# mvenouziou/Boosted_DETR

Measured on AMD Instinct MI355X. Metric: images/sec training step (fwd+matcher+loss+bwd), 640x640 N=100, higher is better.
Workload: dtype f32 (conv/GEMM products as 3 split-f16 [fwd] / split-bf16 [grad] MFMA products, f32 accumulate)

## Files before the change

### boosted_detr_amd/_lib.py

```python
from __future__ import annotations

import ctypes as C
import os
from pathlib import Path

_LIB_PATH = Path(os.environ.get("BDETR_LIB") or Path(__file__).resolve().parent / "csrc" / "libbdetr.so")
_lib = None

c_f32p = C.c_void_p
c_i32p = C.c_void_p
c_i64p = C.c_void_p
c_stream = C.c_void_p


class ConvDesc(C.Structure):
    _fields_ = [(n, C.c_int) for n in ("N", "H", "W", "C", "K", "R", "S", "stride", "pad", "OH", "OW")]


class GemmDesc(C.Structure):
    _fields_ = [
        ("I", C.c_int), ("J", C.c_int), ("R", C.c_int), ("nb0", C.c_int), ("nb1", C.c_int),
        ("a", C.c_void_p), ("lda", C.c_int64), ("sa0", C.c_int64), ("sa1", C.c_int64), ("a_rcontig", C.c_int),
        ("b", C.c_void_p), ("ldb", C.c_int64), ("sb0", C.c_int64), ("sb1", C.c_int64), ("b_rcontig", C.c_int),
        ("c", C.c_void_p), ("ldc", C.c_int64), ("sc0", C.c_int64), ("sc1", C.c_int64),
# ... 12 lines not shown
                ("y2", C.c_void_p), ("mean2", C.c_void_p), ("rstd2", C.c_void_p), ("part_gx2", C.c_void_p)]


class RowchainFwdDesc(C.Structure):
    _fields_ = ([("M", C.c_int64), ("nstages", C.c_int), ("eps", C.c_float), ("rate", C.c_float), ("ctx", C.c_void_p), ("resid", C.c_void_p),
                 ("w", C.c_void_p * 3), ("bias", C.c_void_p * 3)]
                + [(n, C.c_void_p) for n in ("g1", "b1", "g2", "b2", "pre1", "x1", "mean1", "rstd1", "h", "pre2", "x2", "mean2", "rstd2")]
                + [("seed1", C.c_uint64), ("seed2", C.c_uint64), ("seed_base", C.c_void_p)])


class RowchainBwdDesc(C.Structure):
    _fields_ = ([("M", C.c_int64), ("nstages", C.c_int), ("rate", C.c_float)]
                + [(n, C.c_void_p) for n in ("dout", "pre2", "mean2", "rstd2", "g2", "h", "pre1", "mean1", "rstd1", "g1")]
                + [("wt", C.c_void_p * 3)]
                + [(n, C.c_void_p) for n in ("G2", "G1", "G0", "dresid", "dctx", "partials")]
                + [("seed1", C.c_uint64), ("seed2", C.c_uint64), ("seed_base", C.c_void_p)])


class LossDesc(C.Structure):
    _fields_ = [("B", C.c_int), ("M", C.c_int), ("N", C.c_int), ("C", C.c_int), ("A", C.c_int),
                ("category_weight", C.c_float), ("attribute_weight", C.c_float),
                ("box_weight", C.c_float), ("exist_weight", C.c_float)]


P = C.c_void_p
I = C.c_int
L = C.c_int64
F = C.c_float
U64 = C.c_uint64

SIGNATURES = {
    "bdetr_abi_version": (I, []),
    "bdetr_last_error": (C.c_char_p, []),
    "bdetr_device_cus": (I, []),
    "bdetr_low_priority_stream_create": (I, [P]),
    "bdetr_side_stream_candidates": (I, [P, I, I, I, P, P, P]),
    "bdetr_stream_destroy": (I, [P]),
    "bdetr_stream_priority_range": (I, [P, P]),
    "bdetr_set_gemm_precision": (I, [I]),
    "bdetr_get_gemm_precision": (I, []),
    "bdetr_prof_enable": (I, [I]),
    "bdetr_prof_read": (I, [P, P, P]),
    "bdetr_prof_read_arith": (I, [I, P, P, P]),
    "bdetr_prof_dump": (I, [C.c_char_p]),
    "bdetr_image_prep": (I, [P, I, I, I, P, I, I, P]),
    "bdetr_tokens_prepare": (I, [P, P, L, I, I, I, P, P, P]),
    "bdetr_augment_ws_floats": (I, [I]),
    "bdetr_augment": (I, [P, P, P, P, I, I, I, P, P]),
    "bdetr_jpeg_quality_ws_bytes": (C.c_int64, [I, I, I]),
    "bdetr_jpeg_quality": (I, [P, P, P, I, I, I, P, P]),
    "bdetr_augment_jpeg": (I, [P, P, P, P, P, I, I, I, P, P, P]),
    "bdetr_conv2d_fwd": (I, [P, P, P, P, C.POINTER(ConvDesc), I, P, P, P]),
    "bdetr_conv2d_fwd_stat_chunks": (I, [C.POINTER(ConvDesc)]),
    "bdetr_conv2d_bwd_data": (I, [P, P, P, C.POINTER(ConvDesc), I, P]),
    "bdetr_conv2d_bwd_weight": (I, [P, P, P, C.POINTER(ConvDesc), I, P]),
    "bdetr_conv2d_bwd_weight_splitk": (I, [C.POINTER(ConvDesc)]),
    "bdetr_bn_apply_p16": (I, [P, P, P, P, P, P, I, C.POINTER(BnAffine), I, P, P, P, P, P, L, I, P]),
    "bdetr_bn_bwd_p16": (I, [P, P, I, P, P, P, P, P, I, I, P, P, P, P, P, P, P, P, I, L, I, P]),
    "bdetr_bn_bwd_p16_even_pixels": (I, [P, P, I, P, P, P, P, P, I, I, P, P, P, P, P, P, I, I, I, I, I, P]),
    "bdetr_p16_supported": (I, [C.POINTER(ConvDesc)]),
    "bdetr_p16_pack": (I, [P, L, P, P, P, P]),
    "bdetr_p16_unpack": (I, [P, I, L, P, P]),
    "bdetr_p16_pack_conv_weights": (I, [P, I, I, I, I, P, P, P, P]),
    "bdetr_p16_pack_conv_weights_multi": (I, [P, I, P, P]),
    "bdetr_p16_conv2d_fwd_stat_chunks": (I, [C.POINTER(ConvDesc)]),
    "bdetr_p16_conv2d_fwd": (I, [P, P, P, P, C.POINTER(ConvDesc), I, P, P, P]),
    "bdetr_p16_conv2d_bwd_data": (I, [P, P, P, C.POINTER(ConvDesc), I, P]),
    "bdetr_p16_conv2d_bwd_data_stat_chunks": (I, [C.POINTER(ConvDesc)]),
    "bdetr_p16_conv2d_bwd_data_masked_accum": (I, [P, P, P, P, C.POINTER(ConvDesc), C.POINTER(BnBwdFuse), P]),
    "bdetr_p16_conv2d_bwd_data_masked_accum_compact": (I, [P, P, P, P, P, C.POINTER(ConvDesc), C.POINTER(BnBwdFuse), P]),
    "bdetr_relu_mask_apply": (I, [P, P, C.c_int64, P]),
    "bdetr_p16_conv2d_bwd_data_bnstats": (I, [P, P, P, C.POINTER(ConvDesc), C.POINTER(BnBwdFuse), P]),
    "bdetr_p16_conv2d_bwd_weight_splitk": (I, [C.POINTER(ConvDesc)]),
    "bdetr_p16_conv2d_bwd_weight": (I, [P, P, P, C.POINTER(ConvDesc), I, P]),
    "bdetr_p16_conv2d_bwd_weight_xf16": (I, [P, P, P, C.POINTER(ConvDesc), I, P]),
    "bdetr_gemm": (I, [C.POINTER(GemmDesc), P]),
    "bdetr_gemm_ws": (I, [C.POINTER(GemmDesc), P, L, P]),
    "bdetr_splitk_workspace_elems": (L, [L, L, I]),
    "bdetr_conv2d_bwd_weight_ws": (I, [P, P, P, C.POINTER(ConvDesc), I, P, L, P]),
    "bdetr_p16_conv2d_bwd_weight_ws": (I, [P, I, P, P, C.POINTER(ConvDesc), I, P, L, P]),
    "bdetr_gemm_grouped": (I, [C.POINTER(GemmDesc), I, P]),
    "bdetr_colsum_chunks": (I, [L]),
    "bdetr_colsum": (I, [P, L, I, P, P, P]),
    "bdetr_colsum_accumulate": (I, [P, L, I, P, P]),
    "bdetr_colsum_accumulate_group": (I, [P, P, I, P, I, P]),
    "bdetr_colstats": (I, [P, L, I, P, P, P]),
    "bdetr_bn_stats": (I, [P, L, I, P, P, I, F, F, I, P, P, P, P, P, P, P]),
    "bdetr_flag_nonfinite": (I, [P, L, P, P]),
    "bdetr_flag_snapshot": (I, [P, P, P, I, P]),
    "bdetr_debug_checksum": (I, [P, L, P, P, P, I, U64, P]),
    "bdetr_graph_node_census": (I, [P, P, I]),
    "bdetr_bn_stats_fold_rows": (I, []),
    "bdetr_bn_stats_frozen": (I, [P, P, I, F, P, P, P]),
    "bdetr_bn_apply": (I, [P, P, P, P, P, P, I, P, L, I, P]),
    "bdetr_bn_bwd_chunks": (I, [L]),
    "bdetr_bn_bwd": (I, [P, P, P, P, P, P, P, I, I, P, P, P, P, P, L, I, P]),
    "bdetr_bn_rows_stats": (I, [P, I, L, I, F, P, P, P, P, P]),
    "bdetr_bn_rows_apply": (I, [P, P, P, P, P, P, I, L, I, I, P, F, P, P, P, P]),
    "bdetr_bn_rows_bwd": (I, [P, P, P, P, P, I, I, P, P, P, P, I, L, I, P]),
    "bdetr_maxpool3x3s2_fwd": (I, [P, P, I, I, I, I, I, I, P]),
    "bdetr_maxpool3x3s2_bwd": (I, [P, P, P, P, I, I, I, I, I, I, P]),
    "bdetr_stem_pool_bwd_chunks": (I, [L]),
    "bdetr_stem_pool_fwd": (I, [P, P, P, P, P, I, I, I, I, P, P, P, P, P]),
    "bdetr_stem_pool_bwd": (I, [P, P, P, P, P, P, P, I, I, I, I, P, I, P, P, P, P]),
    "bdetr_p16_s2d_pack_bf16": (I, [P, I, I, I, P, P]),
    "bdetr_p16_stem_bwd_weight": (I, [P, P, P, I, I, I, I, P]),
# ... 101 lines not shown
```

### boosted_detr_amd/csrc/igemm.hip

```cpp
#include "gemm_common.h"
#include <stdlib.h>
#include <string.h>
#include <type_traits>
#include <utility>
#include <vector>

using namespace bdgemm;

namespace {

constexpr int BK = 32;
constexpr int RPAD = 4;
constexpr int NTHREADS = 256;

constexpr int SLD = 36;
constexpr int SLD3 = 52;
constexpr float LO_SCALE = 2048.f;
typedef __bf16 bf16x2 __attribute__((ext_vector_type(2)));
typedef __bf16 bf16x8 __attribute__((ext_vector_type(8)));
typedef _Float16 f16x2 __attribute__((ext_vector_type(2)));
typedef _Float16 f16x8 __attribute__((ext_vector_type(8)));
typedef float f32x2 __attribute__((ext_vector_type(2)));

template <int ARITH>
__device__ __forceinline__ void split2(float x0, float x1, unsigned& hi, unsigned& lo) {
    f32x2 v; v[0] = x0; v[1] = x1;
    if (ARITH == AR_BF16X3) {
        hi = __builtin_bit_cast(unsigned, __builtin_convertvector(v, bf16x2));
        f32x2 r;
        r[0] = x0 - __builtin_bit_cast(float, hi << 16);
        r[1] = x1 - __builtin_bit_cast(float, hi & 0xFFFF0000u);
        lo = __builtin_bit_cast(unsigned, __builtin_convertvector(r, bf16x2));
    } else {
        const f16x2 h = __builtin_convertvector(v, f16x2);
        hi = __builtin_bit_cast(unsigned, h);
        const f32x2 r = (v - __builtin_convertvector(h, f32x2)) * LO_SCALE;
        lo = __builtin_bit_cast(unsigned, __builtin_convertvector(r, f16x2));
    }
}

__device__ __forceinline__ void split3(float x0, float x1, unsigned& hi, unsigned& mid, unsigned& lo) {
    f32x2 v; v[0] = x0; v[1] = x1;
    hi = __builtin_bit_cast(unsigned, __builtin_convertvector(v, bf16x2));
    f32x2 r;
    r[0] = x0 - __builtin_bit_cast(float, hi << 16);
    r[1] = x1 - __builtin_bit_cast(float, hi & 0xFFFF0000u);
    mid = __builtin_bit_cast(unsigned, __builtin_convertvector(r, bf16x2));
    r[0] -= __builtin_bit_cast(float, mid << 16);
    r[1] -= __builtin_bit_cast(float, mid & 0xFFFF0000u);
    lo = __builtin_bit_cast(unsigned, __builtin_convertvector(r, bf16x2));
}

struct DenseOp { const float* p; int64_t ld, s0, s1; int rows, cols; };
// ... 358 lines not shown
#pragma unroll
            for (int e = 0; e < 4; ++e)
#pragma unroll
                for (int a = 0; a < TM; ++a)
#pragma unroll
                    for (int b = 0; b < TN; ++b)
                        acc[a][b] = __builtin_amdgcn_mfma_f32_32x32x2f32(fa[a][e], fb[b][e], acc[a][b], 0, 0, 0);
        }
    };

    const int nk = (r_end - r_begin + BK - 1) / BK;
    constexpr bool PF1 = SPLIT && BM * BN >= 128 * 128;
    if constexpr (PF1) {
        if (nk > 0) { load_stage(r_begin, stA0, stB0); write_stage(0, stA0, stB0); }
        __syncthreads();
        for (int kt = 0; kt < nk; ++kt) {
            if (kt + 1 < nk) load_stage(r_begin + (kt + 1) * BK, stA0, stB0);
            compute(kt & 1);
            if (kt + 1 < nk) write_stage((kt + 1) & 1, stA0, stB0);
            __syncthreads();
        }
    } else {
    if (nk > 0) {
        load_stage(r_begin, stA0, stB0);
        if (nk > 1) load_stage(r_begin + BK, stA1, stB1);
        write_stage(0, stA0, stB0);
    }
    __syncthreads();

    for (int kt = 0; kt < nk; kt += 2) {
        if (kt + 2 < nk) load_stage(r_begin + (kt + 2) * BK, stA0, stB0);
        compute(0);
        if (kt + 1 < nk) write_stage(1, stA1, stB1);
        __syncthreads();
        if (kt + 1 >= nk) break;
        if (kt + 3 < nk) load_stage(r_begin + (kt + 3) * BK, stA1, stB1);
        compute(1);
        if (kt + 2 < nk) write_stage(0, stA0, stB0);
        __syncthreads();
    }
    }

    if constexpr (ARITH == AR_FP16X3) {
#pragma unroll
        for (int a = 0; a < TM; ++a)
#pragma unroll
            for (int b = 0; b < TN; ++b)
#pragma unroll
                for (int e = 0; e < 16; ++e) acc[a][b][e] += acc2[a][b][e] * (1.f / LO_SCALE);
    }
    gemm_epilogue<BM, BN, WM, WN, NTHREADS, 2 * STAGE_FLOATS>(acc, g, lds, tile_i, i0, j0, g.c + (int64_t)(sk_ ? zz_ : b0) * g.sc0 + (int64_t)b1 * g.sc1);
}

struct TileChoice { int bm, bn; };

}

namespace bdgemm {
int g_num_cus = 0;
int num_cus() {
    if (g_num_cus == 0) {
        int dev = 0; hipDeviceProp_t p;
        if (hipGetDevice(&dev) == hipSuccess && hipGetDeviceProperties(&p, dev) == hipSuccess) g_num_cus = p.multiProcessorCount;
        if (g_num_cus <= 0) g_num_cus = 256;
    }
    return g_num_cus;
}
}

namespace {

}
namespace bdgemm {
thread_local int g_gemm_mode = -1;
int gemm_mode() {
    if (g_gemm_mode < 0) {
        const char* e = getenv("BDETR_GEMM_PRECISION");
        g_gemm_mode = !e ? BDETR_GEMM_MIXED : (!strcmp(e, "fp32") || !strcmp(e, "f32")) ? BDETR_GEMM_FP32
                    : !strcmp(e, "bf16x3") ? BDETR_GEMM_BF16X3 : !strcmp(e, "split") ? BDETR_GEMM_SPLIT : !strcmp(e, "bf16x6") ? BDETR_GEMM_BF16X6 : BDETR_GEMM_MIXED;
    }
    return g_gemm_mode;
}
}
namespace {
int use_split(bool grad) {
    switch (gemm_mode()) {
        case BDETR_GEMM_FP32:   return AR_FP32;
        case BDETR_GEMM_BF16X3: return AR_BF16X3;
        case BDETR_GEMM_SPLIT:  return grad ? AR_BF16X3 : AR_FP16X3;
        case BDETR_GEMM_BF16X6: return AR_BF16X6;
        default:                return grad ? AR_BF16X3 : AR_FP32;
    }
}

TileChoice choose_tile(int I, int J, int zdim, bool both_rc, bool split, bool patch = false) {
    static int forced_bm = -1, forced_bn = -1;
    if (forced_bm < 0) {
        forced_bm = forced_bn = 0;
        if (const char* e = getenv("BDETR_TILE")) sscanf(e, "%dx%d", &forced_bm, &forced_bn);
    }
    if (forced_bm > 0) {
        if (J <= 32) return {128, 32};
        return {forced_bm, forced_bn};
    }
    auto tiles = [&](int bm, int bn) { return cdiv64(I, bm) * cdiv64(J, bn) * zdim; };
    if (J <= 32) return {128, 32};
// ... 261 lines not shown
            if (arc && brc)   return launch_any<DenseLoader<4>, true, DenseLoader<4>, true>(a, b, g, zdim, st, sp);
            if (arc && !brc)  return launch_any<DenseLoader<4>, true, DenseLoader<4>, false>(a, b, g, zdim, st, sp);
            if (!arc && !brc) return launch_any<DenseLoader<4>, false, DenseLoader<4>, false>(a, b, g, zdim, st, sp);
            return launch_any<DenseLoader<4>, false, DenseLoader<4>, true>(a, b, g, zdim, st, sp, true);
        }
        if (arc && brc)   return launch_any<DenseLoader<1>, true, DenseLoader<1>, true>(a, b, g, zdim, st, AR_FP32, true);
        if (arc && !brc)  return launch_any<DenseLoader<1>, true, DenseLoader<1>, false>(a, b, g, zdim, st, AR_FP32, true);
        if (!arc && !brc) return launch_any<DenseLoader<1>, false, DenseLoader<1>, false>(a, b, g, zdim, st, AR_FP32, true);
        return launch_any<DenseLoader<1>, false, DenseLoader<1>, true>(a, b, g, zdim, st, AR_FP32, true);
    };
    if (ws != nullptr && splitk > 1) return with_splitk_slabs(g, zdim, ws, ws_elems, st, "bdetr_gemm_ws", launch);
    return launch();
}

static int check_conv(const bdetr_conv_desc* d, const char* who) {
    BDETR_CHECK_ARG(d != nullptr, "%s: null desc", who);
    BDETR_CHECK_ARG(d->N > 0 && d->H > 0 && d->W > 0 && d->C > 0 && d->K > 0 && d->R > 0 && d->S > 0 && d->stride > 0 && d->pad >= 0,
                    "%s: bad conv geometry", who);
    BDETR_CHECK_ARG(d->C % 4 == 0, "%s: input channels must be a multiple of 4 (got %d)", who, d->C);
    BDETR_CHECK_ARG(d->OH == (d->H + 2 * d->pad - d->R) / d->stride + 1 && d->OW == (d->W + 2 * d->pad - d->S) / d->stride + 1,
                    "%s: OH/OW inconsistent with geometry", who);
    BDETR_CHECK_ARG((int64_t)d->N * d->OH * d->OW < (1LL << 31) && (int64_t)d->R * d->S * d->C < (1LL << 31), "%s: problem too large", who);
    BDETR_CHECK_ARG(span_ok((int64_t)d->N * d->H * d->W * d->C) && span_ok((int64_t)d->N * d->OH * d->OW * d->K) && span_ok((int64_t)d->K * d->R * d->S * d->C),
                    "%s: a tensor spans 4 GB or more (the loaders use 32-bit buffer offsets); use a smaller per-GPU batch", who);
    return 0;
}

extern "C" int bdetr_conv2d_fwd_stat_chunks(const bdetr_conv_desc* d) {
    if (check_conv(d, "bdetr_conv2d_fwd_stat_chunks")) return -1;
    return stat_chunks(d->N * d->OH * d->OW, d->K);
}

extern "C" int bdetr_conv2d_fwd(const float* x, const float* w, const float* bias, float* y,
                                const bdetr_conv_desc* d, int act, float* stat_sum, float* stat_sq, void* stream) {
    if (int e = check_conv(d, "bdetr_conv2d_fwd")) return e;
    BDETR_CHECK_ARG(x && w && y, "bdetr_conv2d_fwd: null pointer");
    BDETR_CHECK_ARG(aligned16(x) && aligned16(w), "bdetr_conv2d_fwd: x and w must be 16-byte aligned");
    BDETR_CHECK_ARG((stat_sum == nullptr) == (stat_sq == nullptr), "bdetr_conv2d_fwd: stat_sum/stat_sq must both be set or both null");
    const int M = d->N * d->OH * d->OW, Kd = d->R * d->S * d->C;
    GemmParams g; init_params(g);
    g.I = M; g.J = d->K; g.R = Kd;
    g.c = y; g.ldc = d->K; g.bias = bias; g.act = act;
    g.stat_sum = stat_sum; g.stat_sq = stat_sq;
    DenseOp wop{w, Kd, 0, 0, d->K, Kd};
    hipStream_t st = (hipStream_t)stream;
    if (d->R == 1 && d->S == 1 && d->stride == 1 && d->pad == 0) {
        DenseOp xop{x, d->C, 0, 0, M, d->C};
        return launch_any<DenseLoader<4>, true, DenseLoader<4>, true>(xop, wop, g, 1, st, use_split(false));
    }
    PatchOp xop{x, d->N, d->H, d->W, d->C, d->OH, d->OW, d->R, d->S, d->stride, d->pad, M, Kd};
    return launch_any<PatchLoader, true, DenseLoader<4>, true>(xop, wop, g, 1, st, use_split(false));
}

extern "C" int bdetr_conv2d_bwd_data(const float* dy, const float* w, float* dx,
                                     const bdetr_conv_desc* d, int accumulate, void* stream) {
    if (int e = check_conv(d, "bdetr_conv2d_bwd_data")) return e;
    BDETR_CHECK_ARG(dy && w && dx, "bdetr_conv2d_bwd_data: null pointer");
    BDETR_CHECK_ARG(d->K % 4 == 0, "bdetr_conv2d_bwd_data: output channels must be a multiple of 4");
    hipStream_t st = (hipStream_t)stream;
    const int M = d->N * d->OH * d->OW;
    GemmParams g; init_params(g);
    g.c = dx; g.ldc = d->C; g.mode = accumulate ? ST_ACCUM : ST_STORE;
    if (d->R == 1 && d->S == 1 && d->pad == 0) {
        g.I = M; g.J = d->C; g.R = d->K;
        if (d->stride > 1) {
            if (!accumulate) {
                if (int e = bdetr_zero_bytes(dx, sizeof(float) * (size_t)d->N * d->H * d->W * d->C, st)) return e;
            }
            g.rowmap = 1; g.rm_OW = d->OW; g.rm_OHOW = d->OH * d->OW; g.rm_H = d->H; g.rm_W = d->W; g.rm_stride = d->stride;
        }
        DenseOp a{dy, d->K, 0, 0, M, d->K};
        DenseOp b{w, d->C, 0, 0, d->K, d->C};
        return launch_any<DenseLoader<4>, true, DenseLoader<4>, false>(a, b, g, 1, st, use_split(true));
    }
    if (d->stride > 1 && d->pad == 0 && d->R <= d->stride && d->S <= d->stride) {
        if (!accumulate) {
            if (int e = bdetr_zero_bytes(dx, sizeof(float) * (size_t)d->N * d->H * d->W * d->C, st)) return e;
        }
        g.I = M; g.J = d->C; g.R = d->K;
        g.rowmap = 1; g.rm_OW = d->OW; g.rm_OHOW = d->OH * d->OW; g.rm_H = d->H; g.rm_W = d->W; g.rm_stride = d->stride;
        DenseOp a{dy, d->K, 0, 0, M, d->K};
        for (int r = 0; r < d->R; ++r)
            for (int s = 0; s < d->S; ++s) {
                g.rm_off = r * d->W + s;
                DenseOp b{w + (int64_t)(r * d->S + s) * d->C, (int64_t)d->R * d->S * d->C, 0, 0, d->K, d->C};
                if (int e = launch_any<DenseLoader<4>, true, DenseLoader<4>, false>(a, b, g, 1, st, use_split(true))) return e;
            }
        return 0;
    }
    BDETR_CHECK_ARG(d->stride == 1, "bdetr_conv2d_bwd_data: stride>1 only for 1x1 convs or taps that do not overlap (R, S <= stride, pad 0)");
    const int Mx = d->N * d->H * d->W;
    g.I = Mx; g.J = d->C; g.R = d->R * d->S * d->K;
    PatchOp a{dy, d->N, d->OH, d->OW, d->K, d->H, d->W, d->R, d->S, 1, d->R - 1 - d->pad, Mx, d->R * d->S * d->K};
    BDETR_CHECK_ARG(d->R == d->S, "bdetr_conv2d_bwd_data: square kernels only");
    WFlipOp b{w, d->K, d->C, d->R, d->S, d->R * d->S * d->K, d->C};
    return launch_any<PatchLoader, true, WFlipLoader, false>(a, b, g, 1, st, use_split(true));
}

extern "C" int bdetr_conv2d_bwd_weight_splitk(const bdetr_conv_desc* d) {
    if (check_conv(d, "bdetr_conv2d_bwd_weight_splitk")) return -1;
    const int M = d->N * d->OH * d->OW, Kd = d->R * d->S * d->C;
    TileChoice t = choose_tile(d->K, Kd, 2, false, use_split(true) != AR_FP32, !(d->R == 1 && d->S == 1 && d->stride == 1 && d->pad == 0));
    int64_t tiles = cdiv64(d->K, t.bm) * cdiv64(Kd, t.bn);
    int64_t want = 3LL * num_cus();
    const bool few_tiles = tiles <= 8 && M >= (1 << 20);
    if (few_tiles) want = 16LL * num_cus();
// ... 43 lines not shown
```

### boosted_detr_amd/kernels.py

```python
from __future__ import annotations

import ctypes as C
from dataclasses import dataclass
from typing import Optional, Tuple

import numpy as np
import torch

from . import _lib
from ._lib import BnAffine, BnBwdFuse, ConvDesc, GemmDesc, LossDesc, RowchainBwdDesc, RowchainFwdDesc, check

ACT_NONE, ACT_RELU, ACT_TANH = 0, 1, 2


_LAUNCH_STREAM = [None]


def set_launch_stream(handle: Optional[int]) -> Optional[int]:
    prev = _LAUNCH_STREAM[0]
    _LAUNCH_STREAM[0] = handle
    return prev


GEMM_FP32, GEMM_BF16X3, GEMM_MIXED, GEMM_SPLIT, GEMM_BF16X6 = 0, 1, 2, 3, 4
# ... 124 lines not shown
    _chk(image)
    _chk(quality, dtype=torch.int32)
    B, H, W, c = image.shape
    assert c == 3 and quality.numel() == B
    L = _lib.lib()
    out = torch.empty_like(image)
    jws = torch.empty(int(L.bdetr_jpeg_quality_ws_bytes(B, H, W)), dtype=torch.uint8, device=image.device)
    check(L.bdetr_jpeg_quality(_p(image), _p(out), _p(quality), B, H, W, _p(jws), _stream()), "jpeg_quality")
    return out


@dataclass(frozen=True)
class ConvGeom:
    N: int
    H: int
    W: int
    C: int
    K: int
    R: int
    S: int
    stride: int
    pad: int

    @property
    def OH(self) -> int:
        return (self.H + 2 * self.pad - self.R) // self.stride + 1

    @property
    def OW(self) -> int:
        return (self.W + 2 * self.pad - self.S) // self.stride + 1

    @property
    def M(self) -> int:
        return self.N * self.OH * self.OW

    def desc(self) -> ConvDesc:
        return ConvDesc(self.N, self.H, self.W, self.C, self.K, self.R, self.S, self.stride, self.pad, self.OH, self.OW)


def conv2d_fwd(x, w, bias, g: ConvGeom, act: int = ACT_NONE, want_stats: bool = False):
    _chk(x, w, bias)
    L = _lib.lib()
    d = g.desc()
    y = empty(g.N, g.OH, g.OW, g.K, like=x)
    psum = psq = None
    nparts = 0
    if want_stats:
        nparts = L.bdetr_conv2d_fwd_stat_chunks(C.byref(d))
        if nparts <= 0:
            check(-1, "conv2d_fwd_stat_chunks")
        psum = empty(nparts, g.K, like=x)
        psq = empty(nparts, g.K, like=x)
    check(L.bdetr_conv2d_fwd(_p(x), _p(w), _p(bias), _p(y), C.byref(d), act, _p(psum), _p(psq), _stream()), "conv2d_fwd")
    return y, (psum, psq, nparts)


def conv2d_bwd_data(dy, w, g: ConvGeom, dx: Optional[torch.Tensor] = None, accumulate: bool = False):
    _chk(dy, w, dx)
    d = g.desc()
    if dx is None:
        assert not accumulate
        dx = empty(g.N, g.H, g.W, g.C, like=dy)
    check(_lib.lib().bdetr_conv2d_bwd_data(_p(dy), _p(w), _p(dx), C.byref(d), int(accumulate), _stream()), "conv2d_bwd_data")
    return dx


def conv2d_bwd_weight(x, dy, g: ConvGeom, dw: Optional[torch.Tensor] = None, prezeroed: bool = False):
    _chk(x, dy, dw)
    L = _lib.lib()
    d = g.desc()
    if dw is None:
        dw = empty(g.K, g.R, g.S, g.C, like=x)
        prezeroed = False
    sk = L.bdetr_conv2d_bwd_weight_splitk(C.byref(d))
    if sk > 1 and not prezeroed:
        check(L.bdetr_zero(_p(dw), dw.numel(), _stream()), "zero")
    ws, n = _splitk_ws(g.K, g.R * g.S * g.C, sk, x)
    check(L.bdetr_conv2d_bwd_weight_ws(_p(x), _p(dy), _p(dw), C.byref(d), sk, _p(ws), n, _stream()), "conv2d_bwd_weight")
    return dw


_OVERFLOW = [None]


def overflow_flag() -> torch.Tensor:
    if _OVERFLOW[0] is None:
        _OVERFLOW[0] = torch.zeros(1, dtype=torch.int32, device="cuda")
    return _OVERFLOW[0]


_GUARD_ACTIVE = [True]


def set_guard_active(on: bool) -> None:
    _GUARD_ACTIVE[0] = bool(on)


def flag_nonfinite(x: torch.Tensor) -> None:
    _chk(x)
    check(_lib.lib().bdetr_flag_nonfinite(_p(x), x.numel(), _p(overflow_flag()), _stream()), "flag_nonfinite")


def flag_snapshot(ordinal: torch.Tensor, host_ring: torch.Tensor) -> None:
    assert host_ring.dtype == torch.int32 and host_ring.numel() >= 2 and host_ring.is_pinned()
    assert ordinal.dtype == torch.int32 and ordinal.is_cuda
    check(_lib.lib().bdetr_flag_snapshot(_p(overflow_flag()), _p(ordinal), host_ring.data_ptr(), host_ring.numel() - 1, _stream()), "flag_snapshot")
# ... 1229 lines not shown
```

### boosted_detr_amd/ops.py

```python
from __future__ import annotations

import math
import os
import weakref
from typing import Optional

import numpy as np
import torch

from . import kernels as K
from . import _lib
from .engine import WEIGHTS_VERSION, Variable, capture, current_tape, dense_contribution, info, materialise, own, side_task, tag

_dropout_site = [0]
_dropout_seed_dev = [None]


def dropout_seed_tensor() -> torch.Tensor:
    if _dropout_seed_dev[0] is None:
        _dropout_seed_dev[0] = torch.full((1,), 0x5EED, dtype=torch.int64, device="cuda")
    return _dropout_seed_dev[0]


def set_dropout_seed(seed: int, write: bool = True) -> None:
# ... 433 lines not shown
    def backward(g_out):
        dx, _ = _bn_backward(_2d(g_out.contiguous()), None, x2d, mean, rstd, bn, False, not training, False)
        return (own(dx.view(x.shape)),)

    _rec([out], [x], backward)
    return out


def batchnorm_rows(x: torch.Tensor, bn: BNState, training: bool, groups: int) -> torch.Tensor:
    x2d = _2d(x)
    g, b = bn.gamma.value, bn.beta.value
    if training:
        mean, rstd, var = K.bn_rows_stats(x2d, groups, bn.eps)
        out2d = K.bn_rows_apply(x2d, groups, mean, rstd, g, b, var, bn.momentum, bn.moving_mean.value, bn.moving_var.value)
    else:
        K.demote_split_forward()
        mean, rstd = K.bn_stats_frozen(bn.moving_mean.value, bn.moving_var.value, bn.eps)
        out2d = K.bn_rows_apply(x2d, groups, mean, rstd, g, b)
    out = out2d.view(x.shape)

    def backward(g_out):
        sg, sb = GradSink(bn.gamma), GradSink(bn.beta)
        dx, _, _ = K.bn_rows_bwd(_2d(g_out.contiguous()), x2d, groups, mean, rstd, bn.gamma.value, not training, dgamma=sg.buf, dbeta=sb.buf)
        sg.commit()
        sb.commit()
        return (own(dx.view(x.shape)),)

    _rec([out], [x], backward)
    return out


def stack_rows(xs) -> torch.Tensor:
    L, B = len(xs), xs[0].shape[0]
    out = torch.empty((L * B,) + tuple(xs[0].shape[1:]), dtype=xs[0].dtype, device=xs[0].device)
    for l, x in enumerate(xs):
        K.copy_cols(x.contiguous(), x.shape[-1], out[l * B:(l + 1) * B], 0)

    def backward(g):
        g, mine = g.contiguous(), info(g).owned
        return tuple(own(g[l * B:(l + 1) * B]) if mine else g[l * B:(l + 1) * B] for l in range(L))

    _rec([out], list(xs), backward)
    return out


def maxpool(x: torch.Tensor) -> torch.Tensor:
    y = K.maxpool_fwd(x)
    _rec([y], [x], lambda g: (own(K.maxpool_bwd(x, y, g.contiguous())),))
    return y


STEM_FUSE = os.environ.get("BDETR_STEM_FUSE", "1") != "0"
STEM_S2D = os.environ.get("BDETR_STEM_S2D", "1") != "0"


def conv_bn_relu_maxpool(x: torch.Tensor, w: Variable, b: Variable, bn: BNState, stride: int, pad: int, training: bool,
                         bn_batch_stats: bool) -> torch.Tensor:
    N, H, W, Cin = x.shape
    Kout, R, S, _ = w.value.shape
    if not (STEM_FUSE and training and bn_batch_stats and _p16_active() and Kout % 8 == 0):
        return maxpool(conv_bn(x, w, b, bn, stride, pad, True, training=training, bn_batch_stats=bn_batch_stats, x_needs_grad=False))
    g = K.ConvGeom(N, H, W, Cin, Kout, R, S, stride, pad)
    x32 = as_fp32(x)
    y, parts = K.conv2d_fwd(x32, w.value, b.value, g, K.ACT_NONE, want_stats=True)
    if parts is None or parts[0] is None:
        parts = K.colstats(_2d(y))
    mean, rstd = K.bn_stats(g.M, Kout, parts, bn.eps, bn.momentum, True, bn.moving_mean.value, bn.moving_var.value, like=y)
    _, out, tap = K.stem_pool_fwd(y, mean, rstd, bn.gamma.value, bn.beta.value)
    attach_packed(out, out.detach(), p16_only=True)

    def backward(g_out):
        sg, sb = GradSink(bn.gamma), GradSink(bn.beta)
        s2d = (STEM_S2D and w.needs_grad and (R, S, stride, pad, Cin) == (7, 7, 2, 3, 4) and H % 2 == 0 and W % 2 == 0 and Kout % 64 == 0
               and K.get_gemm_precision() in ("split", "mixed") and not K.deterministic())
        dy, _, _ = K.stem_pool_bwd(materialise(g_out).contiguous(), tap, y, mean, rstd, bn.gamma.value, bn.beta.value, dgamma=sg.buf, dbeta=sb.buf,
                                   dy_p16=s2d)
        sg.commit()
        sb.commit()
        if s2d:
            _param_grads_task(w, b, lambda dw, pz: K.stem_bwd_weight_s2d(x32, dy, dw), None, x32, dy)
        else:
            _param_grads_task(w, b, lambda dw, pz: K.conv2d_bwd_weight(x32, dy, g, dw=dw, prezeroed=pz), None, x32, dy)
        return (None,)

    _rec([out], [x], backward)
    return out


def dense(x: torch.Tensor, w: Variable, b: Variable, act: int = K.ACT_NONE) -> torch.Tensor:
    x2d = _2d(x)
    y2d = K.linear_fwd(x2d, w.value, b.value, act)
    y = y2d.view(*x.shape[:-1], w.value.shape[0])

    def backward(g_out, acc=None):
        g2d = _2d(g_out.contiguous())
        if act == K.ACT_RELU:
            g2d = K.relu_bwd(y2d, g2d)
        elif act == K.ACT_TANH:
            g2d = K.tanh_bwd(y2d, g2d)
        _param_grads_task(w, b, lambda dw, pz: K.linear_bwd_weight(g2d, x2d, dw=dw, prezeroed=pz), g2d, x2d, g2d)
        have = acc[0] if acc is not None else None
        if have is not None and have.is_contiguous() and have.shape == x.shape:
            K.linear_bwd_data(g2d, w.value, dx=_2d(materialise(have)), accumulate=True)
            dense_contribution(have)
            return (have,)
        return (own(K.linear_bwd_data(g2d, w.value).view(x.shape)),)

    backward.wants_acc = True
    _rec([y], [x], backward)
    return y


def dense_group(xs, ws, bs):
    x2 = [_2d(x) for x in xs]
    aligned = all(t.data_ptr() % 16 == 0 for t in x2) and x2[0].shape[1] % 4 == 0 and ws[0].value.shape[0] % 4 == 0
    same = all(w.value.shape == ws[0].value.shape for w in ws)
    if not (aligned and same) or len(xs) > 4:
# ... 257 lines not shown
```

### include/bdetr.h

```cpp
#ifndef BDETR_H
#define BDETR_H
#include <stdint.h>
#ifdef __cplusplus
extern "C" {
#endif

#define BDETR_ABI_VERSION 8

int         bdetr_abi_version(void);
const char* bdetr_last_error(void);
int         bdetr_device_cus(void);

int         bdetr_low_priority_stream_create(void** stream_out);
int         bdetr_stream_priority_range(int* least, int* greatest);
int         bdetr_side_stream_candidates(void* main_stream, int ncand, int loads, int ticks, void** streams_out, float* scores_ms, float* unloaded_ms);
int         bdetr_stream_destroy(void* stream);

enum { BDETR_GEMM_FP32 = 0, BDETR_GEMM_BF16X3 = 1, BDETR_GEMM_MIXED = 2, BDETR_GEMM_SPLIT = 3, BDETR_GEMM_BF16X6 = 4 };
int         bdetr_set_gemm_precision(int mode);
int         bdetr_get_gemm_precision(void);

int bdetr_prof_enable(int on);
int bdetr_prof_read(double* total_ms, int64_t* launches, double* flops);
int bdetr_prof_read_arith(int arith, double* total_ms, int64_t* launches, double* flops);
int bdetr_prof_dump(const char* path);

enum { BDETR_ACT_NONE = 0, BDETR_ACT_RELU = 1, BDETR_ACT_TANH = 2 };

int bdetr_image_prep(const float* in, int B, int h, int w, float* out, int H, int W, void* stream);

int bdetr_tokens_prepare(const int* cat_ids, const int* att_ids, int64_t rows, int slots, int C, int A,
                         int* cat_out, float* att_hot, void* stream);

int bdetr_augment_ws_floats(int B);
int bdetr_augment(const float* in, float* out, const int32_t* iparams, const float* fparams,
                  int B, int H, int W, float* ws, void* stream);
int64_t bdetr_jpeg_quality_ws_bytes(int B, int H, int W);
int bdetr_jpeg_quality(const float* in, float* out, const int32_t* quality, int B, int H, int W, void* ws, void* stream);
int bdetr_augment_jpeg(const float* in, float* out, const int32_t* iparams, const float* fparams, const int32_t* quality,
                       int B, int H, int W, float* ws, void* jpeg_ws, void* stream);

typedef struct {
    int N, H, W, C;
    int K, R, S;
    int stride, pad;
    int OH, OW;
} bdetr_conv_desc;

int bdetr_conv2d_fwd(const float* x, const float* w, const float* bias, float* y,
                     const bdetr_conv_desc* d, int act, float* stat_sum, float* stat_sq, void* stream);
int bdetr_conv2d_fwd_stat_chunks(const bdetr_conv_desc* d);
int bdetr_conv2d_bwd_data(const float* dy, const float* w, float* dx,
                          const bdetr_conv_desc* d, int accumulate, void* stream);
int bdetr_conv2d_bwd_weight(const float* x, const float* dy, float* dw,
                            const bdetr_conv_desc* d, int splitk, void* stream);
int bdetr_conv2d_bwd_weight_splitk(const bdetr_conv_desc* d);
int bdetr_conv2d_bwd_weight_ws(const float* x, const float* dy, float* dw,
                               const bdetr_conv_desc* d, int splitk, float* ws, int64_t ws_elems, void* stream);
int64_t bdetr_splitk_workspace_elems(int64_t I, int64_t J, int splitk);

typedef struct { const float* mean; const float* rstd; const float* gamma; const float* beta; } bdetr_bn_affine;
int bdetr_bn_apply_p16(const float* x, const float* mean, const float* rstd, const float* gamma,
                       const float* beta, const void* residual, int residual_p16, const bdetr_bn_affine* residual_bn, int relu, float* out32,
                       void* out_f16, void* out_bf16, uint64_t* relu_mask, int* overflow_flag, int64_t rows, int C,
                       void* stream);
int bdetr_bn_bwd_p16(const float* dout, const void* out, int out_p16, const float* x, const float* mean,
                     const float* rstd, const float* gamma, const float* beta, int relu, int frozen,
                     float* dx32, void* dx_bf16, float* dgamma, float* dbeta, float* dresidual,
                     float* ws, const float* pre_g, const float* pre_gx, int pre_n, int64_t rows, int C, void* stream);
int bdetr_bn_bwd_p16_even_pixels(const float* dout, const void* out, int out_p16, const float* x, const float* mean,
                                 const float* rstd, const float* gamma, const float* beta, int relu, int frozen,
                                 float* dx32, void* dx_bf16, float* dgamma, float* dbeta, float* dresidual,
                                 float* ws, int N, int H, int W, int C,
                                 int dout_compact , void* stream);
int bdetr_p16_supported(const bdetr_conv_desc* d);
int bdetr_p16_pack(const float* x, int64_t n, void* f16_out, void* bf16_out, int* overflow_flag, void* stream);
int bdetr_p16_unpack(const void* p, int is_f16, int64_t n, float* out, void* stream);
int bdetr_p16_pack_conv_weights(const float* w, int K, int R, int S, int C, void* w_f16, void* wt_bf16,
                                int* overflow_flag, void* stream);
int bdetr_p16_pack_conv_weights_multi(const int64_t* table, int ntensors, int* overflow_flag, void* stream);
int bdetr_p16_conv2d_fwd_stat_chunks(const bdetr_conv_desc* d);
int bdetr_p16_conv2d_fwd(const void* x_f16, const void* w_f16, const float* bias, float* y,
                         const bdetr_conv_desc* d, int act, float* stat_sum, float* stat_sq, void* stream);
int bdetr_p16_conv2d_bwd_data(const void* dy_bf16, const void* wt_bf16, float* dx,
                              const bdetr_conv_desc* d, int accumulate, void* stream);
typedef struct {
    const float* y; const float* mean; const float* rstd; const float* gamma; const float* beta; int relu;
    float* part_g; float* part_gx;
    const uint64_t* relu_mask;
    const float* y2; const float* mean2; const float* rstd2; float* part_gx2;
} bdetr_bn_bwd_fuse;
int bdetr_p16_conv2d_bwd_data_stat_chunks(const bdetr_conv_desc* d);
int bdetr_relu_mask_apply(float* x, const uint64_t* relu_mask, int64_t n, void* stream);
int bdetr_p16_conv2d_bwd_data_masked_accum(const void* dy_bf16, const void* wt_bf16, float* dx, const uint64_t* relu_mask,
                                           const bdetr_conv_desc* d, const bdetr_bn_bwd_fuse* bn , void* stream);
int bdetr_p16_conv2d_bwd_data_masked_accum_compact(const void* dy_bf16, const void* wt_bf16, float* dx, const float* old_even,
                                                   const uint64_t* relu_mask, const bdetr_conv_desc* d, const bdetr_bn_bwd_fuse* bn, void* stream);
int bdetr_p16_conv2d_bwd_data_bnstats(const void* dy_bf16, const void* wt_bf16, float* dx,
                                      const bdetr_conv_desc* d, const bdetr_bn_bwd_fuse* bn, void* stream);
int bdetr_p16_conv2d_bwd_weight_splitk(const bdetr_conv_desc* d);
int bdetr_p16_conv2d_bwd_weight(const void* x_bf16, const void* dy_bf16, float* dw,
                                const bdetr_conv_desc* d, int splitk, void* stream);
int bdetr_p16_conv2d_bwd_weight_xf16(const void* x_f16, const void* dy_bf16, float* dw,
                                     const bdetr_conv_desc* d, int splitk, void* stream);
// ... 240 lines not shown
```

Measured before the change: 645.7.

## Add windowed stem conv kernel that reuses input rows in LDS

Adds a dedicated 7x7/stride-2 stem convolution forward kernel that stages a shared input window per output tile in LDS, plus all 7 weight K-tiles resident, instead of the generic im2col patch loader. Tiles are distributed per XCD in a persistent loop with double-buffered register prefetch of the next window. The aim is to cut redundant global loads of overlapping patches in the stem forward. It adds a specialised code path with a fit check and falls back to the generic conv otherwise.

```diff
diff --git a/boosted_detr_amd/_lib.py b/boosted_detr_amd/_lib.py
--- a/boosted_detr_amd/_lib.py
+++ b/boosted_detr_amd/_lib.py
@@ -88,6 +88,8 @@
     "bdetr_augment_jpeg": (I, [P, P, P, P, P, I, I, I, P, P, P]),
     "bdetr_conv2d_fwd": (I, [P, P, P, P, C.POINTER(ConvDesc), I, P, P, P]),
     "bdetr_conv2d_fwd_stat_chunks": (I, [C.POINTER(ConvDesc)]),
+    "bdetr_stem_conv2d_fwd": (I, [P, P, P, P, C.POINTER(ConvDesc), I, P, P, P]),
+    "bdetr_stem_conv2d_fwd_fits": (I, [C.POINTER(ConvDesc)]),
     "bdetr_conv2d_bwd_data": (I, [P, P, P, C.POINTER(ConvDesc), I, P]),
     "bdetr_conv2d_bwd_weight": (I, [P, P, P, C.POINTER(ConvDesc), I, P]),
     "bdetr_conv2d_bwd_weight_splitk": (I, [C.POINTER(ConvDesc)]),
diff --git a/boosted_detr_amd/csrc/igemm.hip b/boosted_detr_amd/csrc/igemm.hip
--- a/boosted_detr_amd/csrc/igemm.hip
+++ b/boosted_detr_amd/csrc/igemm.hip
@@ -1,4 +1,5 @@
 #include "gemm_common.h"
+#include <algorithm>
 #include <stdlib.h>
 #include <string.h>
 #include <type_traits>
@@ -463,6 +464,177 @@
     gemm_epilogue<BM, BN, WM, WN, NTHREADS, 2 * STAGE_FLOATS>(acc, g, lds, tile_i, i0, j0, g.c + (int64_t)(sk_ ? zz_ : b0) * g.sc0 + (int64_t)b1 * g.sc1);
 }
 
+constexpr int WIN_NSEG = 12;
+constexpr int WIN_P = 64 + 3 * WIN_NSEG;
+constexpr int WIN_DW = 14 * WIN_P * 4;
+constexpr int STEM_NK = 7;
+
+struct StemOp { const float* p; int N, H, W, OH, OW; };
+
+constexpr int stem_tap_off(int t) {
+    return t < 49 ? (((t / 7) * 2 + ((t % 7) & 1)) * WIN_P + ((t % 7) >> 1)) * 4 : 0;
+}
+
+template <int ARITH>
+__global__ __launch_bounds__(NTHREADS, 2)
+void stem_window_kernel(StemOp opa, DenseOp opb, GemmParams g)
+{
+    static_assert(ARITH == AR_FP16X3 || ARITH == AR_BF16X3, "two-term splits only");
+    constexpr int BM = 64, BN = 64, WM = 2, WN = 2, NK = STEM_NK, NVB = BN * BK / 4 / NTHREADS;
+    constexpr int B_DW = BN * 32;
+    static_assert(BM * (BN + 4) <= WIN_DW, "the epilogue's padded tile aliases the window");
+    __shared__ __attribute__((aligned(16))) float lds[WIN_DW + NK * B_DW];
+    unsigned* win = reinterpret_cast<unsigned*>(lds);
+    unsigned* bres = win + WIN_DW;
+
+    const int tid = threadIdx.x;
+    const int lane = tid & 63;
+    const int wave = tid >> 6;
+    const int wm = wave / WN, wn = wave % WN;
+    const int li = lane & 31, lh = lane >> 5;
+
+    const int nper = (int)gridDim.x >> 3, xcd = (int)blockIdx.x & 7;
+    const int q8 = g.tiles_i >> 3, r8 = g.tiles_i & 7;
+    const int t_first = (xcd < r8 ? xcd * (q8 + 1) : r8 * (q8 + 1) + (xcd - r8) * q8) + ((int)blockIdx.x >> 3);
+    const int t_last = (xcd < r8 ? (xcd + 1) * (q8 + 1) : r8 * (q8 + 1) + (xcd + 1 - r8) * q8);
+    if (t_first >= t_last) return;
+    const int j0 = (int)blockIdx.y * BN;
+    const int OW = opa.OW;
+
+    const __amdgpu_buffer_rsrc_t rsA = make_rsrc(opa.p);
+    const __amdgpu_buffer_rsrc_t rsB = make_rsrc(opb.p);
+    g.mode = ST_STORE; g.rowmap = 0; g.bnb_y = nullptr; g.alpha = 1.f;
+    float bias_pre[1];
+    gemm_load_bias<BM, BN, WM, WN>(g, j0, bias_pre);
+
+    {
+        const int b_cols = min(opb.cols, g.R);
+#pragma unroll 1
+        for (int kt = 0; kt < NK; ++kt) {
+            f32x4 rb[NVB];
+#pragma unroll
+            for (int p = 0; p < NVB; ++p) {
+                const int e = tid + NTHREADS * p, row = e >> 3, col = kt * BK + 4 * (e & 7);
+                rb[p] = buf_load4(rsB, (j0 + row < opb.rows && col < b_cols) ? ((unsigned)(j0 + row) * (unsigned)opb.ld + (unsigned)col) * 4u : OOB);
+            }
+#pragma unroll
+            for (int p = 0; p < NVB; ++p) {
+                const int e = tid + NTHREADS * p, row = e >> 3, c4 = e & 7;
+                const int w = (((c4 >> 1) ^ ((row >> 1) & 7)) << 2) | ((c4 & 1) << 1);
+                unsigned* dst = bres + kt * B_DW + row * 32;
+                unsigned h0, l0, h1, l1;
+                split2<ARITH>(rb[p][0], rb[p][1], h0, l0);
+                split2<ARITH>(rb[p][2], rb[p][3], h1, l1);
+                u32x2 hi, lo;
+                hi[0] = h0; hi[1] = h1; lo[0] = l0; lo[1] = l1;
+                *reinterpret_cast<u32x2*>(dst + w) = hi;
+                *reinterpret_cast<u32x2*>(dst + (w ^ 16)) = lo;
+            }
+        }
+    }
+    const int slot = tid >> 1, plane = tid & 1;
+    f32x4 va[7], vb[7];
+    bool used_a = false, used_b = false;
+    auto load_window = [&](int tile_i, f32x4 (&v)[7], bool& used) {
+        const int i0 = tile_i * BM, i_end = min(i0 + BM, g.I);
+        const int g0 = i0 / OW, ow0 = i0 - g0 * OW;
+        const int n0 = OW - ow0;
+        int k = 0, c = slot;
+        if (slot >= n0 + 3) { const int y = slot - (n0 + 3); k = 1 + y / (OW + 3); c = y - (k - 1) * (OW + 3); }
+        const int gk = g0 + k;
+        const int first = k == 0 ? i0 : gk * OW;
+        const int last = min(gk * OW + OW, i_end);
+        used = tile_i < t_last && slot < WIN_P && first < last && c < last - first + 3;
+        const int n = gk / opa.OH, oh = gk - n * opa.OH;
+        const int iw = 2 * ((k == 0 ? ow0 : 0) + c) - 3 + plane;
+        const int ih0 = 2 * oh - 3;
+        const bool col_ok = used && (unsigned)iw < (unsigned)opa.W;
+        const unsigned base = (unsigned)((n * opa.H + ih0) * opa.W + iw) * 16u;
+#pragma unroll
+        for (int r = 0; r < 7; ++r)
+            v[r] = buf_load4(rsA, (col_ok && (unsigned)(ih0 + r) < (unsigned)opa.H) ? base + (unsigned)(r * opa.W) * 16u : OOB);
+    };
+    load_window(t_first, va, used_a);
+    load_window(t_first + nper, vb, used_b);
+
+    const int xbB = wn * 32 + li;
+    const unsigned* brow = bres + xbB * 32;
+    const int bswz = (xbB >> 1) & 7;
+    constexpr bool TWO_ACC = ARITH == AR_FP16X3;
+
+    auto run_tile = [&](int tile_i, f32x4 (&v)[7], bool& used) {
+        const int i0 = tile_i * BM, i_end = min(i0 + BM, g.I);
+        if (used) {
+#pragma unroll
+            for (int r = 0; r < 7; ++r) {
+                unsigned h0, l0, h1, l1;
+                split2<ARITH>(v[r][0], v[r][1], h0, l0);
+                split2<ARITH>(v[r][2], v[r][3], h1, l1);
+                u32x4 px;
+                px[0] = h0; px[1] = h1; px[2] = l0; px[3] = l1;
+                *reinterpret_cast<u32x4*>(win + ((r * 2 + plane) * WIN_P + slot) * 4) = px;
+            }
+        }
+        __syncthreads();
+        load_window(tile_i + 2 * nper, v, used);
+
+        const int ia = min(i0 + wm * 32 + li, i_end - 1);
+        const unsigned* arow = win + ((ia - i0) + 3 * (ia / OW - i0 / OW)) * 4;
+
+        f32x16 acc[1][1], acc2;
+#pragma unroll
+        for (int e = 0; e < 16; ++e) { acc[0][0][e] = 0.f; acc2[e] = 0.f; }
+#pragma unroll
+        for (int kt = 0; kt < NK; ++kt) {
+            const unsigned* qB = brow + kt * B_DW;
+#pragma unroll
+            for (int ks = 0; ks < BK / 16; ++ks) {
+                const int t0 = kt * 8 + ks * 4;
+                u32x4 v0 = {0u, 0u, 0u, 0u}, v1 = v0;
+                if (t0 < 49) {
+                    v0 = *reinterpret_cast<const u32x4*>(arow + (lh ? stem_tap_off(t0 + 2) : stem_tap_off(t0)));
+                    if (t0 + 2 >= 49 && lh) v0 = u32x4{0u, 0u, 0u, 0u};
+                }
+                if (t0 + 1 < 49) {
+                    v1 = *reinterpret_cast<const u32x4*>(arow + (lh ? stem_tap_off(t0 + 3) : stem_tap_off(t0 + 1)));
+                    if (t0 + 3 >= 49 && lh) v1 = u32x4{0u, 0u, 0u, 0u};
+                }
+                u32x4 ah, al;
+                ah[0] = v0[0]; ah[1] = v0[1]; ah[2] = v1[0]; ah[3] = v1[1];
+                al[0] = v0[2]; al[1] = v0[3]; al[2] = v1[2]; al[3] = v1[3];
+                const int w = ((ks * 2 + lh) ^ bswz) << 2;
+                const u32x4 bh = *reinterpret_cast<const u32x4*>(qB + w);
+                const u32x4 bl = *reinterpret_cast<const u32x4*>(qB + (w ^ 16));
+                if constexpr (TWO_ACC) {
+#define H8(v) __builtin_bit_cast(f16x8, v)
+                    acc2 = __builtin_amdgcn_mfma_f32_32x32x16_f16(H8(al), H8(bh), acc2, 0, 0, 0);
+                    acc2 = __builtin_amdgcn_mfma_f32_32x32x16_f16(H8(ah), H8(bl), acc2, 0, 0, 0);
+                    acc[0][0] = __builtin_amdgcn_mfma_f32_32x32x16_f16(H8(ah), H8(bh), acc[0][0], 0, 0, 0);
+#undef H8
+                } else {
+#define BF8(v) __builtin_bit_cast(bf16x8, v)
+                    acc[0][0] = __builtin_amdgcn_mfma_f32_32x32x16_bf16(BF8(al), BF8(bh), acc[0][0], 0, 0, 0);
+                    acc[0][0] = __builtin_amdgcn_mfma_f32_32x32x16_bf16(BF8(ah), BF8(bl), acc[0][0], 0, 0, 0);
+                    acc[0][0] = __builtin_amdgcn_mfma_f32_32x32x16_bf16(BF8(ah), BF8(bh), acc[0][0], 0, 0, 0);
+#undef BF8
+                }
+            }
+        }
+        if constexpr (TWO_ACC) {
+#pragma unroll
+            for (int e = 0; e < 16; ++e) acc[0][0][e] += acc2[e] * (1.f / LO_SCALE);
+        }
+        gemm_epilogue<BM, BN, WM, WN, NTHREADS, WIN_DW>(acc, g, lds, tile_i, i0, j0, g.c, bias_pre);
+        __syncthreads();
+    };
+    int tile_i = t_first;
+    for (; tile_i + nper < t_last; tile_i += 2 * nper) {
+        run_tile(tile_i, va, used_a);
+        run_tile(tile_i + nper, vb, used_b);
+    }
+    if (tile_i < t_last) run_tile(tile_i, va, used_a);
+}
+
 struct TileChoice { int bm, bn; };
 
 }
@@ -830,6 +1002,53 @@
     return launch_any<PatchLoader, true, DenseLoader<4>, true>(xop, wop, g, 1, st, use_split(false));
 }
 
+static bool stem_window_fits(const bdetr_conv_desc* d) {
+    if (!(d->R == 7 && d->S == 7 && d->stride == 2 && d->pad == 3 && d->C == 4 && d->K % 64 == 0)) return false;
+    const int arith = use_split(false);
+    if (arith != AR_FP16X3 && arith != AR_BF16X3) return false;
+    const int M = d->N * d->OH * d->OW;
+    const TileChoice t = choose_tile(M, d->K, 1, true, true, true);
+    if (t.bm != 64 || t.bn != 64) return false;
+    const int64_t nseg = M <= 64 ? cdiv64(M, d->OW) : (64 - 2) / d->OW + 2;
+    return nseg <= WIN_NSEG;
+}
+
+extern "C" int bdetr_stem_conv2d_fwd_fits(const bdetr_conv_desc* d) {
+    if (check_conv(d, "bdetr_stem_conv2d_fwd_fits")) return -1;
+    return stem_window_fits(d) ? 1 : 0;
+}
+
+extern "C" int bdetr_stem_conv2d_fwd(const float* x, const float* w, const float* bias, float* y,
+                                     const bdetr_conv_desc* d, int act, float* stat_sum, float* stat_sq, void* stream) {
+    if (int e = check_conv(d, "bdetr_stem_conv2d_fwd")) return e;
+    BDETR_CHECK_ARG(x && w && y, "bdetr_stem_conv2d_fwd: null pointer");
+    BDETR_CHECK_ARG(aligned16(x) && aligned16(w), "bdetr_stem_conv2d_fwd: x and w must be 16-byte aligned");
+    BDETR_CHECK_ARG((stat_sum == nullptr) == (stat_sq == nullptr), "bdetr_stem_conv2d_fwd: stat_sum/stat_sq must both be set or both null");
+    BDETR_CHECK_ARG(stem_window_fits(d), "bdetr_stem_conv2d_fwd: not a 7x7 / stride 2 / pad 3 convolution of a 4-channel image with K %% 64 == 0 under a "
+                    "split forward arithmetic whose window fits (N=%d H=%d W=%d C=%d K=%d R=%d S=%d stride=%d pad=%d): use bdetr_conv2d_fwd",
+                    d->N, d->H, d->W, d->C, d->K, d->R, d->S, d->stride, d->pad);
+    const int M = d->N * d->OH * d->OW, Kd = d->R * d->S * d->C;
+    GemmParams g; init_params(g);
+    g.I = M; g.J = d->K; g.R = Kd;
+    g.c = y; g.ldc = d->K; g.bias = bias; g.act = act;
+    g.stat_sum = stat_sum; g.stat_sq = stat_sq;
+    g.tiles_i = (int)cdiv64(M, 64);
+    g.tiles_j = d->K / 64;
+    g.vec_store = aligned16(y);
+    StemOp xop{x, d->N, d->H, d->W, d->OH, d->OW};
+    DenseOp wop{w, Kd, 0, 0, d->K, Kd};
+    hipStream_t st = (hipStream_t)stream;
+    const int arith = use_split(false);
+    const bool prof = g_prof_on;
+    if (prof) prof_begin(st, 2.0 * (double)M * (double)d->K * (double)Kd, M, d->K, Kd, 1, 64, 64, arith * 10000 + LoaderId<PatchLoader>::v * 1000 + 100 + 1);
+    const int per_xcd = (int)std::max<int64_t>(1, std::min<int64_t>(cdiv64(g.tiles_i, 8), 2 * num_cus() / 8));
+    const dim3 grid(8 * per_xcd, g.tiles_j);
+    if (arith == AR_FP16X3) hipLaunchKernelGGL(stem_window_kernel<AR_FP16X3>, grid, dim3(NTHREADS), 0, st, xop, wop, g);
+    else                    hipLaunchKernelGGL(stem_window_kernel<AR_BF16X3>, grid, dim3(NTHREADS), 0, st, xop, wop, g);
+    if (prof) prof_end(st);
+    return bdetr_launch_status("stem_window");
+}
+
 extern "C" int bdetr_conv2d_bwd_data(const float* dy, const float* w, float* dx,
                                      const bdetr_conv_desc* d, int accumulate, void* stream) {
     if (int e = check_conv(d, "bdetr_conv2d_bwd_data")) return e;
diff --git a/boosted_detr_amd/kernels.py b/boosted_detr_amd/kernels.py
--- a/boosted_detr_amd/kernels.py
+++ b/boosted_detr_amd/kernels.py
@@ -200,6 +200,28 @@
         psum = empty(nparts, g.K, like=x)
         psq = empty(nparts, g.K, like=x)
     check(L.bdetr_conv2d_fwd(_p(x), _p(w), _p(bias), _p(y), C.byref(d), act, _p(psum), _p(psq), _stream()), "conv2d_fwd")
+    return y, (psum, psq, nparts)
+
+
+def stem_conv2d_fwd_fits(g: ConvGeom) -> bool:
+    d = g.desc()
+    return _lib.lib().bdetr_stem_conv2d_fwd_fits(C.byref(d)) == 1
+
+
+def stem_conv2d_fwd(x, w, bias, g: ConvGeom, act: int = ACT_NONE, want_stats: bool = False):
+    _chk(x, w, bias)
+    L = _lib.lib()
+    d = g.desc()
+    y = empty(g.N, g.OH, g.OW, g.K, like=x)
+    psum = psq = None
+    nparts = 0
+    if want_stats:
+        nparts = L.bdetr_conv2d_fwd_stat_chunks(C.byref(d))
+        if nparts <= 0:
+            check(-1, "conv2d_fwd_stat_chunks")
+        psum = empty(nparts, g.K, like=x)
+        psq = empty(nparts, g.K, like=x)
+    check(L.bdetr_stem_conv2d_fwd(_p(x), _p(w), _p(bias), _p(y), C.byref(d), act, _p(psum), _p(psq), _stream()), "stem_conv2d_fwd")
     return y, (psum, psq, nparts)
 
 
diff --git a/boosted_detr_amd/ops.py b/boosted_detr_amd/ops.py
--- a/boosted_detr_amd/ops.py
+++ b/boosted_detr_amd/ops.py
@@ -509,6 +509,7 @@
 
 STEM_FUSE = os.environ.get("BDETR_STEM_FUSE", "1") != "0"
 STEM_S2D = os.environ.get("BDETR_STEM_S2D", "1") != "0"
+STEM_WINDOW = os.environ.get("BDETR_STEM_WINDOW", "1") != "0"
 
 
 def conv_bn_relu_maxpool(x: torch.Tensor, w: Variable, b: Variable, bn: BNState, stride: int, pad: int, training: bool,
@@ -519,7 +520,8 @@
         return maxpool(conv_bn(x, w, b, bn, stride, pad, True, training=training, bn_batch_stats=bn_batch_stats, x_needs_grad=False))
     g = K.ConvGeom(N, H, W, Cin, Kout, R, S, stride, pad)
     x32 = as_fp32(x)
-    y, parts = K.conv2d_fwd(x32, w.value, b.value, g, K.ACT_NONE, want_stats=True)
+    stem_fwd = K.stem_conv2d_fwd if STEM_WINDOW and K.stem_conv2d_fwd_fits(g) else K.conv2d_fwd
+    y, parts = stem_fwd(x32, w.value, b.value, g, K.ACT_NONE, want_stats=True)
     if parts is None or parts[0] is None:
         parts = K.colstats(_2d(y))
     mean, rstd = K.bn_stats(g.M, Kout, parts, bn.eps, bn.momentum, True, bn.moving_mean.value, bn.moving_var.value, like=y)
diff --git a/include/bdetr.h b/include/bdetr.h
--- a/include/bdetr.h
+++ b/include/bdetr.h
@@ -50,6 +50,9 @@
 int bdetr_conv2d_fwd(const float* x, const float* w, const float* bias, float* y,
                      const bdetr_conv_desc* d, int act, float* stat_sum, float* stat_sq, void* stream);
 int bdetr_conv2d_fwd_stat_chunks(const bdetr_conv_desc* d);
+int bdetr_stem_conv2d_fwd(const float* x, const float* w, const float* bias, float* y,
+                          const bdetr_conv_desc* d, int act, float* stat_sum, float* stat_sq, void* stream);
+int bdetr_stem_conv2d_fwd_fits(const bdetr_conv_desc* d);
 int bdetr_conv2d_bwd_data(const float* dy, const float* w, float* dx,
                           const bdetr_conv_desc* d, int accumulate, void* stream);
 int bdetr_conv2d_bwd_weight(const float* x, const float* dy, float* dw,
```

Result: no change. 649.2, median of 6 (+0.5%).
